# gusanagy/Hybrid-Diffusion-Underwater-Atmopheric-Image-Enhancement

Hardware: AMD Instinct MI355X
Metric: denoising-steps/sec (256x256, T=1000) (higher is better)
Workload: dtype f32 (tensors and accumulation fp32; every operand of the attention contractions as 2xfp16 pieces -- scores: a balance per product term, four terms at d_head 16 / three at d_head 32; P.V: three terms -- and of the 3x3 convs behind GroupNorm likewise (other 3x3 convs: 3xbf16 pieces), on the 16-bit MFM

## Files before the change

### hybrid-diffusion-underwater-atmopheric-image-enhancement_amd/csrc/conv3x3_x3.hip

```cpp
#include <stdlib.h>

#include <type_traits>

#include "common.h"
#include "conv_x3.h"
#include "device.h"

using namespace hdiff;

namespace {

constexpr int THREADS = 256;
constexpr int PH = 10, PW = 34, PPIX = PH * PW;
constexpr int NSLOT = (4 * PPIX + THREADS - 1) / THREADS;
constexpr int HALF_WORDS = PPIX * 4;
constexpr int PIECE_WORDS = 2 * HALF_WORDS;
constexpr int PSTRIDE = PIECE_WORDS + 8;
constexpr int DUMP_WORD = PIECE_WORDS;


__device__ constexpr int TERM_W[6] = {2, 1, 0, 1, 0, 0};
__device__ constexpr int TERM_X[6] = {0, 1, 2, 0, 1, 0};

template <int NT, bool OUTMAP, bool PAIR, int OCC = 1, bool DROP = false>
__global__ __launch_bounds__(THREADS, OCC) void conv3x3_x3_kernel(const ConvX3K p) {
  constexpr int NP = PAIR ? 2 : 3;
  __shared__ __attribute__((aligned(16))) unsigned sXbuf[2][NP * PSTRIDE];
  extern __shared__ __attribute__((aligned(16))) float sG[];

  const int tid = threadIdx.x, lane = tid & 63, wave = tid >> 6;
  const int l31 = lane & 31, h = lane >> 5;
  const int b = blockIdx.z;
  int tile_id = blockIdx.x, cob = blockIdx.y;
  if ((gridDim.x & 7u) == 0u && gridDim.y > 1u) {
    const unsigned lin = blockIdx.x + gridDim.x * blockIdx.y, per = 8u * gridDim.y;
    const unsigned grp = lin / per, r = lin - grp * per;
    tile_id = (int)(grp * 8u + (r & 7u));
    cob = (int)(r >> 3);
  }
  const int co0 = cob * 64;
  const int tile_y = tile_id / p.tiles_x, tile_x = tile_id - tile_y * p.tiles_x;
  const int vy0 = tile_y * 8, vx0 = tile_x * 32;
  const bool has_gn = p.gn_scale != nullptr;
  const size_t HW = (size_t)p.H * p.W;
  const size_t IHW = (size_t)p.IH * p.IW;
  float xs = 1.0f, xinv = 1.0f;
  if constexpr (PAIR) {
    if (p.absmax_in != nullptr) {
      int e = (int)((p.absmax_in[b] >> 23) & 0xffu) - 127;
      e = e < -100 ? -100 : (e > 127 ? 127 : e);
      xs = __builtin_bit_cast(float, (unsigned)(14 - e + 127) << 23);
      xinv = __builtin_bit_cast(float, (unsigned)(e - 14 + 127) << 23);
    } else {
      xs = p.act_scale[0];
      xinv = p.act_scale[1];
    }
  }
  const float one = p.one;

  int s_goff[NSLOT];
  int s_lds[NSLOT];
  int s_quad[NSLOT];
#pragma unroll
  for (int i = 0; i < NSLOT; ++i) {
    const int e = tid + i * THREADS;
    const int jq = e / PPIX, pos = e - jq * PPIX;
    const int py = pos / PW, px = pos - py * PW;
    const int iy = vy0 - 1 + py, ix = vx0 - 1 + px;
    const bool used = jq < 4;
    s_quad[i] = used ? jq : 3;
    s_lds[i] = used ? (jq >> 1) * HALF_WORDS + pos * 4 + (jq & 1) * 2 : DUMP_WORD;
    const int gy = iy * p.in_s + p.in_oy, gx = ix * p.in_s + p.in_ox;
    s_goff[i] = (used && iy >= 0 && gy < p.IH && ix >= 0 && gx < p.IW) ? gy * p.IW + gx : -1;
  }
  if (has_gn) {
    for (int i = tid; i < 2 * p.Cin; i += THREADS)
      sG[i] = (i < p.Cin) ? p.gn_scale[b * p.Cin + i] : p.gn_shift[b * p.Cin + (i - p.Cin)];
  }

  const int wm = wave & 1, wn = wave >> 1;
  f32x16 acc[4];
#pragma unroll
  for (int nt = 0; nt < 4; ++nt)
#pragma unroll
    for (int r = 0; r < 16; ++r) acc[nt][r] = 0.f;

  constexpr bool XAHEAD = PAIR;
  f32x4 xv[NSLOT], xv2[XAHEAD ? NSLOT : 1];
  unsigned kw[DROP ? 4 : 1];
  unsigned ksh = 0;
  auto fetch_keep = [&](int i, int c0, unsigned tie) {
    if constexpr (DROP) {
      const unsigned hw = (unsigned)IHW;
      unsigned e = (unsigned)(b * p.Cin + c0 + 4 * s_quad[i]) * hw + (unsigned)(s_goff[i] >= 0 ? s_goff[i] : 0);
      asm("" : "+v"(e) : "v"(tie));
      ksh = 0;
#pragma unroll
      for (int k = 0; k < 4; ++k) {
        kw[k] = p.keep_bits[e >> 5];
        ksh |= (e & 31u) << (5 * k);
        e += hw;
      }
    }
  };
  auto issue_loads_to = [&](f32x4 (&dst)[XAHEAD ? NSLOT : 1], int c0) {
    const float* xbase = (c0 < p.C0) ? p.x0 + ((size_t)b * p.C0 + c0) * IHW : p.x1 + ((size_t)b * p.C1 + (c0 - p.C0)) * IHW;
#pragma unroll
    for (int i = 0; i < (XAHEAD ? NSLOT : 0); ++i) {
      const bool ok = s_goff[i] >= 0;
      const float* src = xbase + (size_t)(4 * s_quad[i]) * IHW + (ok ? s_goff[i] : 0);
      const float v0 = src[0], v1 = src[IHW], v2 = src[2 * IHW], v3 = src[3 * IHW];
      dst[i] = f32x4{ok ? v0 : 0.f, ok ? v1 : 0.f, ok ? v2 : 0.f, ok ? v3 : 0.f};
    }
  };
  auto issue_loads = [&](int c0) {
    const float* xbase = (c0 < p.C0) ? p.x0 + ((size_t)b * p.C0 + c0) * IHW : p.x1 + ((size_t)b * p.C1 + (c0 - p.C0)) * IHW;
#pragma unroll
    for (int i = 0; i < NSLOT; ++i) {
      const bool ok = s_goff[i] >= 0;
      const float* src = xbase + (size_t)(4 * s_quad[i]) * IHW + (ok ? s_goff[i] : 0);
      const float v0 = src[0], v1 = src[IHW], v2 = src[2 * IHW], v3 = src[3 * IHW];
      xv[i] = f32x4{ok ? v0 : 0.f, ok ? v1 : 0.f, ok ? v2 : 0.f, ok ? v3 : 0.f};
    }
  };
  auto stage_slot = [&](auto gn_tag, int i, int c0, unsigned* sX) {
    constexpr bool GN = decltype(gn_tag)::value;
    f32x4 v = xv[i];
    if (GN) {
      const int ci = c0 + 4 * s_quad[i];
      const f32x4 sc = *reinterpret_cast<const f32x4*>(&sG[ci]);
      const f32x4 sh = *reinterpret_cast<const f32x4*>(&sG[p.Cin + ci]);
      const bool inside = s_goff[i] >= 0;
#pragma unroll
      for (int k = 0; k < 4; ++k) {
        if constexpr (DROP) {
          const bool kept = (kw[k] >> ((ksh >> (5 * k)) & 31u)) & 1u;
          v[k] = (inside && kept) ? swish_fast(fmaf(v[k], sc[k], sh[k])) * p.inv_keep : 0.f;
        } else {
          v[k] = inside ? swish_fast(fmaf(v[k], sc[k], sh[k])) : 0.f;
        }
      }
      if constexpr (DROP) {
        const unsigned tie = __builtin_bit_cast(unsigned, v[0]);
        if (i + 1 < NSLOT) fetch_keep(i + 1, c0, tie);
        else fetch_keep(0, c0 + 16 < p.Cin ? c0 + 16 : c0, tie);
      }
    }
    if constexpr (PAIR) {
      unsigned a0, a1, c0w, c1w;
      split2(v[0] * xs, v[1] * xs, one, a0, a1);
      split2(v[2] * xs, v[3] * xs, one, c0w, c1w);
      if (HDIFF_MUTANT & 1) { a1 &= 0xffe0ffe0u; c1w &= 0xffe0ffe0u; }
      *reinterpret_cast<u32x2*>(&sX[s_lds[i]]) = u32x2{a0, c0w};
      *reinterpret_cast<u32x2*>(&sX[PSTRIDE + s_lds[i]]) = u32x2{a1, c1w};
    } else {
      unsigned a0, a1, a2, c0w, c1w, c2w;
      split3(v[0], v[1], a0, a1, a2);
      split3(v[2], v[3], c0w, c1w, c2w);
      *reinterpret_cast<u32x2*>(&sX[s_lds[i]]) = u32x2{a0, c0w};
      *reinterpret_cast<u32x2*>(&sX[PSTRIDE + s_lds[i]]) = u32x2{a1, c1w};
      *reinterpret_cast<u32x2*>(&sX[2 * PSTRIDE + s_lds[i]]) = u32x2{a2, c2w};
    }
  };
  auto store_staged = [&](auto gn_tag, int c0, unsigned* sX) {
#pragma unroll
    for (int i = 0; i < NSLOT; ++i) stage_slot(gn_tag, i, c0, sX);
  };

  int boff[4];
#pragma unroll
  for (int nt = 0; nt < 4; ++nt) boff[nt] = h * HALF_WORDS + ((wn * 4 + nt) * PW + l31) * 4;
  const unsigned* wlane = p.wp3 + ((size_t)(co0 + wm * 32 + l31) * 8 + h * 4);
  const size_t w_piece = (size_t)p.CoutPad * 8;
  const size_t w_tap = NP * w_piece, w_chunk = NT * w_tap;

  auto load_w = [&](u32x4 (&wa)[NP], int chunk, int tap) {
    const unsigned* wb = wlane + (size_t)chunk * w_chunk + (size_t)tap * w_tap;
#pragma unroll
    for (int pc = 0; pc < NP; ++pc) wa[pc] = *reinterpret_cast<const u32x4*>(wb + pc * w_piece);
  };
  auto load_x = [&](u32x4 (&xp)[NP], const unsigned* sX, int tap, int nt) {
    const int toff = p.tap_off[tap];
#pragma unroll
    for (int pc = 0; pc < NP; ++pc) xp[pc] = *reinterpret_cast<const u32x4*>(&sX[pc * PSTRIDE + boff[nt] + toff]);
  };
  auto mma_unit = [&](const u32x4 (&wa)[NP], const u32x4 (&xp)[NP], int nt) {
    if constexpr (PAIR) {
      acc[nt] = mfma_f16(wa[1], xp[0], acc[nt]);
      acc[nt] = mfma_f16(wa[0], xp[1], acc[nt]);
      acc[nt] = mfma_f16(wa[0], xp[0], acc[nt]);
    } else {
#pragma unroll
      for (int t = 0; t < 6; ++t)
        if (!((HDIFF_MUTANT & 1) && TERM_W[t] == 0 && TERM_X[t] == 2)) acc[nt] = mfma_bf16(wa[TERM_W[t]], xp[TERM_X[t]], acc[nt]);
    }
  };

  constexpr bool WSTREAM = (NT % 3 == 0);
  u32x4 w[3][NP];
  auto chunk = [&](auto gn_tag, auto more_tag, int c, int nchunks) {
    constexpr bool more = decltype(more_tag)::value;
    const unsigned* sX = sXbuf[c & 1];
    unsigned* sNext = sXbuf[(c + 1) & 1];
    u32x4 xp[2][NP];
    if (XAHEAD && c + 2 < nchunks) issue_loads_to(xv2, (c + 2) * 16);
    if (!WSTREAM || c == 0) {
      load_w(w[0], c, 0);
      load_w(w[1], c, 1);
    }
    load_x(xp[0], sX, 0, 0);
#pragma unroll
    for (int tap = 0; tap < NT; ++tap) {
      if (tap + 2 < NT) load_w(w[(tap + 2) % 3], c, tap + 2);
      else if (WSTREAM && more) load_w(w[(tap + 2) % 3], c + 1, tap + 2 - NT);
#pragma unroll
      for (int nt = 0; nt < 4; ++nt) {
        const int u = tap * 4 + nt;
        if (u + 1 < 4 * NT) load_x(xp[(u + 1) & 1], sX, (u + 1) / 4, (u + 1) % 4);
        mma_unit(w[tap % 3], xp[u & 1], nt);
      }
      if (more && tap < NSLOT) stage_slot(gn_tag, tap, (c + 1) * 16, sNext);
    }
    if (more) {
#pragma unroll
      for (int i = NT; i < NSLOT; ++i) stage_slot(gn_tag, i, (c + 1) * 16, sNext);
    }
    if constexpr (XAHEAD) {
      if (c + 2 < nchunks) {
#pragma unroll
        for (int i = 0; i < NSLOT; ++i) xv[i] = xv2[i];
      }
    } else {
      if (c + 2 < nchunks) issue_loads((c + 2) * 16);
    }
    __syncthreads();
  };

  const int nchunks = p.Cin / 16;
  issue_loads(0);
  fetch_keep(0, 0, 0u);
  __syncthreads();
  if (has_gn) store_staged(std::true_type{}, 0, sXbuf[0]);
  else store_staged(std::false_type{}, 0, sXbuf[0]);
  if (nchunks > 1) issue_loads(16);
  __syncthreads();
  if (has_gn) {
    for (int c = 0; c + 1 < nchunks; ++c) chunk(std::true_type{}, std::true_type{}, c, nchunks);
    chunk(std::true_type{}, std::false_type{}, nchunks - 1, nchunks);
  } else {
    for (int c = 0; c + 1 < nchunks; ++c) chunk(std::false_type{}, std::true_type{}, c, nchunks);
    chunk(std::false_type{}, std::false_type{}, nchunks - 1, nchunks);
  }

  if constexpr (PAIR) {
    const float os = xinv * p.w_scale[1];
#pragma unroll
    for (int nt = 0; nt < 4; ++nt)
#pragma unroll
      for (int r = 0; r < 16; ++r) acc[nt][r] *= os;
  }
  const size_t OHW = OUTMAP ? (size_t)p.OH * p.OW : HW;
  const int osy = OUTMAP ? p.out_sy : 1, ooy = OUTMAP ? p.out_oy : 0, osx = OUTMAP ? p.out_sx : 1, oox = OUTMAP ? p.out_ox : 0;
  const int OW = OUTMAP ? p.OW : p.W;
  const bool track = p.absmax_out != nullptr;
  unsigned amax = 0u;
  auto post_absmax = [&]() {
    if (!track) return;
#pragma unroll
    for (int o = 32; o > 0; o >>= 1) {
      const unsigned other = (unsigned)__shfl_xor((int)amax, o, 64);
      amax = other > amax ? other : amax;
    }
    if (lane == 0) atomicMax(&p.absmax_out[b], amax);
  };
  if (co0 + 64 <= p.Cout && vy0 + 8 <= p.H && vx0 + 32 <= p.W) {
    float add[16];
#pragma unroll
    for (int r = 0; r < 16; ++r) {
      const int co = co0 + wm * 32 + (r & 3) + 8 * (r >> 2) + 4 * h;
      float a = 0.f;
      if (p.bias) a += p.bias[co];
      if (p.addvec) a += p.addvec[b * p.Cout + co];
      add[r] = a;
    }
    const size_t lane_base = ((size_t)b * p.Cout + co0 + wm * 32 + 4 * h) * OHW +
                             (size_t)((vy0 + wn * 4) * osy + ooy) * OW + (size_t)(vx0 + l31) * osx + oox;
#pragma unroll
    for (int nt = 0; nt < 4; ++nt) {
      const size_t row = lane_base + (size_t)(nt * osy) * OW;
      float res[16];
      if (p.residual) {
#pragma unroll
        for (int r = 0; r < 16; ++r) res[r] = p.residual[row + (size_t)((r & 3) + 8 * (r >> 2)) * OHW];
      }
      float vv[16];
#pragma unroll
      for (int r = 0; r < 16; ++r) {
        float v;
        if (p.residual_first) v = (acc[nt][r] + res[r]) + add[r];
        else {
          v = acc[nt][r] + add[r];
          if (p.residual) v += res[r];
        }
        p.out[row + (size_t)((r & 3) + 8 * (r >> 2)) * OHW] = v;
        vv[r] = v;
      }
      if (track) {
#pragma unroll
        for (int r = 0; r < 16; ++r) {
          const unsigned vb = __builtin_bit_cast(unsigned, vv[r]) & 0x7fffffffu;
          amax = vb > amax ? vb : amax;
        }
      }
    }
    post_absmax();
    return;
  }
#pragma unroll
  for (int nt = 0; nt < 4; ++nt) {
    const int vy = vy0 + wn * 4 + nt, vx = vx0 + l31;
    if (vy >= p.H || vx >= p.W) continue;
    const size_t pix = (size_t)(vy * osy + ooy) * OW + (size_t)vx * osx + oox;
#pragma unroll
    for (int r = 0; r < 16; ++r) {
      const int co = co0 + wm * 32 + (r & 3) + 8 * (r >> 2) + 4 * h;
      if (co < p.Cout) {
        float a = 0.f;
        if (p.bias) a += p.bias[co];
        if (p.addvec) a += p.addvec[b * p.Cout + co];
        const size_t o = ((size_t)b * p.Cout + co) * OHW + pix;
        float v;
        if (p.residual_first) v = (acc[nt][r] + p.residual[o]) + a;
        else {
          v = acc[nt][r] + a;
          if (p.residual) v += p.residual[o];
        }
        p.out[o] = v;
        if (track) {
          const unsigned vb = __builtin_bit_cast(unsigned, v) & 0x7fffffffu;
          amax = vb > amax ? vb : amax;
        }
      }
    }
  }
  post_absmax();
}

struct PackX3K {
  int mode, Cout, Cin, KH, KW, ntaps, CoutPad;
  int CinPad;
  int ky[9], kx[9];
};
__global__ void pack_conv_weight_x3_kernel(const float* __restrict__ w, unsigned* __restrict__ wp3, const PackX3K q) {
  const size_t n = (size_t)(q.Cin / 16) * q.ntaps * q.CoutPad * 8;
  for (size_t i = (size_t)blockIdx.x * blockDim.x + threadIdx.x; i < n; i += (size_t)gridDim.x * blockDim.x) {
    const int j = (int)(i % 8);
    size_t r = i / 8;
    const int co = (int)(r % q.CoutPad);
    r /= q.CoutPad;
    const int tap = (int)(r % q.ntaps);
    const int chunk = (int)(r / q.ntaps);
    float a = 0.f, c = 0.f;
    if (co < q.Cout) {
      const int ci = chunk * 16 + 2 * j;
      const size_t k = (size_t)q.ky[tap] * q.KW + q.kx[tap], kk = (size_t)q.KH * q.KW;
      if (q.mode == 1) {
        a = w[((size_t)ci * q.Cout + co) * kk + k];
        c = w[((size_t)(ci + 1) * q.Cout + co) * kk + k];
      } else {
        a = w[((size_t)co * q.Cin + ci) * kk + k];
        c = w[((size_t)co * q.Cin + ci + 1) * kk + k];
      }
    }
    unsigned h0, h1, h2;
    split3(a, c, h0, h1, h2);
    const size_t base = ((size_t)(chunk * q.ntaps + tap) * 3) * q.CoutPad * 8 + (size_t)co * 8 + j;
    wp3[base] = h0;
    wp3[base + (size_t)q.CoutPad * 8] = h1;
    wp3[base + 2 * (size_t)q.CoutPad * 8] = h2;
  }
}

__global__ void conv_weight_absmax_kernel(const float* __restrict__ w, size_t n, unsigned* __restrict__ tail) {
  float m = 0.f;
  for (size_t i = (size_t)blockIdx.x * blockDim.x + threadIdx.x; i < n; i += (size_t)gridDim.x * blockDim.x) m = fmaxf(m, fabsf(w[i]));
#pragma unroll
  for (int o = 32; o > 0; o >>= 1) m = fmaxf(m, __shfl_xor(m, o, 64));
  if ((threadIdx.x & 63) == 0) atomicMax(tail, __builtin_bit_cast(unsigned, m));
}
__global__ void pack_conv_weight_h2_kernel(const float* __restrict__ w, unsigned* __restrict__ wp2, unsigned* __restrict__ tail,
                                           const PackX3K q, float one) {
  const size_t n = (size_t)(q.Cin / 16) * q.ntaps * q.CoutPad * 8;
  int e = (int)((tail[0] >> 23) & 0xffu) - 127;
  e = e < -60 ? -60 : (e > 60 ? 60 : e);
  const float sc = __builtin_bit_cast(float, (unsigned)(14 - e + 127) << 23);
  for (size_t i = (size_t)blockIdx.x * blockDim.x + threadIdx.x; i < n; i += (size_t)gridDim.x * blockDim.x) {
    const int j = (int)(i % 8);
    size_t r = i / 8;
    const int co = (int)(r % q.CoutPad);
    r /= q.CoutPad;
    const int tap = (int)(r % q.ntaps);
    const int chunk = (int)(r / q.ntaps);
    float a = 0.f, c = 0.f;
    if (co < q.Cout) {
      const int ci = chunk * 16 + 2 * j;
      const size_t k = (size_t)q.ky[tap] * q.KW + q.kx[tap], kk = (size_t)q.KH * q.KW;
      if (q.mode == 2) {
        a = w[(k * q.CinPad + ci) * q.CoutPad + co];
        c = w[(k * q.CinPad + ci + 1) * q.CoutPad + co];
      } else if (q.mode == 1) {
        a = w[((size_t)ci * q.Cout + co) * kk + k];
        c = w[((size_t)(ci + 1) * q.Cout + co) * kk + k];
      } else {
        a = w[((size_t)co * q.Cin + ci) * kk + k];
        c = w[((size_t)co * q.Cin + ci + 1) * kk + k];
      }
    }
    unsigned h0, h1;
    split2(a * sc, c * sc, one, h0, h1);
    const size_t base = ((size_t)(chunk * q.ntaps + tap) * 2) * q.CoutPad * 8 + (size_t)co * 8 + j;
    wp2[base] = h0;
    wp2[base + (size_t)q.CoutPad * 8] = h1;
  }
  if (blockIdx.x == 0 && threadIdx.x == 0) {
    reinterpret_cast<float*>(tail)[1] = __builtin_bit_cast(float, (unsigned)(e - 14 + 127) << 23);
    reinterpret_cast<float*>(tail)[2] = sc;
    tail[3] = 0u;
  }
}

__global__ void gn_act_scale_kernel(const float* __restrict__ gamma, const float* __restrict__ beta, int C, float sqrt_n1,
                                    float gain, float* __restrict__ out) {
  __shared__ float red[4];
  float m = 0.f;
  for (int i = threadIdx.x; i < C; i += blockDim.x) m = fmaxf(m, fmaf(sqrt_n1, fabsf(gamma[i]), fabsf(beta[i])));
#pragma unroll
  for (int o = 32; o > 0; o >>= 1) m = fmaxf(m, __shfl_xor(m, o, 64));
  if ((threadIdx.x & 63) == 0) red[threadIdx.x >> 6] = m;
  __syncthreads();
  if (threadIdx.x == 0) {
    m = fmaxf(fmaxf(red[0], red[1]), fmaxf(red[2], red[3])) * gain;
    int e = (int)((__builtin_bit_cast(unsigned, m) >> 23) & 0xffu) - 127;
    e = e < -60 ? -60 : (e > 60 ? 60 : e);
    out[0] = __builtin_bit_cast(float, (unsigned)(13 - e + 127) << 23);
    out[1] = __builtin_bit_cast(float, (unsigned)(e - 13 + 127) << 23);
  }
}

}

namespace hdiff {

void launch_conv3x3_x3(const ConvX3K& k, int B, hipStream_t stream) {
  const int tiles_y = cdiv(k.H, 8);
  dim3 grid(k.tiles_x * tiles_y, cdiv(k.Cout, 64), B);
  const size_t dyn = (size_t)2 * k.Cin * sizeof(float);
  const bool outmap = !(k.out_sy == 1 && k.out_oy == 0 && k.out_sx == 1 && k.out_ox == 0 && k.OH == k.H && k.OW == k.W);
  if (k.keep_bits != nullptr) {
    if (k.act_scale != nullptr) hipLaunchKernelGGL((conv3x3_x3_kernel<9, false, true, 2, true>), grid, dim3(THREADS), dyn, stream, k);
    else hipLaunchKernelGGL((conv3x3_x3_kernel<9, false, false, 2, true>), grid, dim3(THREADS), dyn, stream, k);
    return;
  }
  if (k.act_scale != nullptr || k.absmax_in != nullptr) {
    if (k.ntaps == 9 && !outmap) hipLaunchKernelGGL((conv3x3_x3_kernel<9, false, true>), grid, dim3(THREADS), dyn, stream, k);
    else if (k.ntaps == 9) hipLaunchKernelGGL((conv3x3_x3_kernel<9, true, true>), grid, dim3(THREADS), dyn, stream, k);
    else if (k.ntaps == 6 && !outmap) hipLaunchKernelGGL((conv3x3_x3_kernel<6, false, true>), grid, dim3(THREADS), dyn, stream, k);
    else if (k.ntaps == 4 && !outmap) hipLaunchKernelGGL((conv3x3_x3_kernel<4, false, true>), grid, dim3(THREADS), dyn, stream, k);
    else if (k.ntaps == 6) hipLaunchKernelGGL((conv3x3_x3_kernel<6, true, true>), grid, dim3(THREADS), dyn, stream, k);
    else hipLaunchKernelGGL((conv3x3_x3_kernel<4, true, true>), grid, dim3(THREADS), dyn, stream, k);
    return;
  }
  if (k.ntaps == 9 && !outmap) hipLaunchKernelGGL((conv3x3_x3_kernel<9, false, false>), grid, dim3(THREADS), dyn, stream, k);
  else if (k.ntaps == 9) hipLaunchKernelGGL((conv3x3_x3_kernel<9, true, false>), grid, dim3(THREADS), dyn, stream, k);
  else if (k.ntaps == 6) hipLaunchKernelGGL((conv3x3_x3_kernel<6, true, false>), grid, dim3(THREADS), dyn, stream, k);
  else hipLaunchKernelGGL((conv3x3_x3_kernel<4, true, false>), grid, dim3(THREADS), dyn, stream, k);
}

}

static int pack_x3(const float* w, void* wp3, int mode, int Cout, int Cin, int KH, int KW, int ntaps, const int* ky, const int* kx,
                   int CoutPad, hipStream_t stream) {
  PackX3K q{};
  q.mode = mode; q.Cout = Cout; q.Cin = Cin; q.KH = KH; q.KW = KW; q.ntaps = ntaps; q.CoutPad = CoutPad;
  for (int t = 0; t < ntaps; ++t) { q.ky[t] = ky[t]; q.kx[t] = kx[t]; }
  const size_t n = (size_t)(Cin / 16) * ntaps * CoutPad * 8;
  const int blocks = (int)((n + 255) / 256 < 4096 ? (n + 255) / 256 : 4096);
  (void)hipGetLastError();
  hipLaunchKernelGGL(pack_conv_weight_x3_kernel, dim3(blocks), dim3(256), 0, stream, w, (unsigned*)wp3, q);
  HDIFF_CHECK_LAUNCH("pack_conv_weight_x3_kernel");
  return HDIFF_OK;
}

extern "C" int hdiff_pack_conv_weight_x3(const float* w, void* wp3, int Cout, int Cin, int CoutPad, int transposed,
                                         hdiff_stream_t stream) {
  HDIFF_CHECK_ARG(w && wp3, "pack_conv_weight_x3: null pointer");
  HDIFF_CHECK_ARG(Cout > 0 && Cin > 0 && Cin % 16 == 0 && CoutPad >= Cout && CoutPad % 64 == 0,
                  "pack_conv_weight_x3: needs Cin %% 16 == 0 and CoutPad %% 64 == 0 (Cin %d, Cout %d, CoutPad %d)", Cin, Cout, CoutPad);
  int ky[9], kx[9];
  for (int t = 0; t < 9; ++t) {
    ky[t] = transposed ? 2 - t / 3 : t / 3;
    kx[t] = transposed ? 2 - t % 3 : t % 3;
  }
  return pack_x3(w, wp3, transposed ? 1 : 0, Cout, Cin, 3, 3, 9, ky, kx, CoutPad, (hipStream_t)stream);
}

extern "C" int hdiff_pack_conv_weight_h2_words(int Cout, int Cin, int CoutPad, int64_t* words_out) {
  HDIFF_CHECK_ARG(words_out, "pack_conv_weight_h2_words: null pointer");
  HDIFF_CHECK_ARG(Cout > 0 && Cin > 0 && Cin % 16 == 0 && CoutPad >= Cout && CoutPad % 64 == 0,
                  "pack_conv_weight_h2_words: needs Cin %% 16 == 0 and CoutPad %% 64 == 0 (Cin %d, Cout %d, CoutPad %d)", Cin, Cout, CoutPad);
  *words_out = (int64_t)(Cin / 16) * 9 * 2 * CoutPad * 8 + 4;
  return HDIFF_OK;
}

static int pack_h2(const char* who, const float* w, void* wp2, int mode, int Cout, int Cin, int KH, int KW, int ntaps, const int* ky,
                   const int* kx, int CoutPad, hipStream_t stream) {
  PackX3K q{};
  q.mode = mode; q.Cout = Cout; q.Cin = Cin; q.KH = KH; q.KW = KW; q.ntaps = ntaps; q.CoutPad = CoutPad;
  for (int t = 0; t < ntaps; ++t) { q.ky[t] = ky[t]; q.kx[t] = kx[t]; }
  const size_t n = (size_t)(Cin / 16) * ntaps * CoutPad * 8, nw = (size_t)Cout * Cin * KH * KW;
  unsigned* tail = (unsigned*)wp2 + 2 * n;
  const int blocks = (int)((n + 255) / 256 < 4096 ? (n + 255) / 256 : 4096);
  const int mblocks = (int)((nw + 255) / 256 < 1024 ? (nw + 255) / 256 : 1024);
  (void)hipGetLastError();
  if (hipMemsetAsync(tail, 0, 16, stream) != hipSuccess) {
    hdiff::set_error("%s: hipMemsetAsync failed", who);
    return HDIFF_ERR_LAUNCH;
  }
  hipLaunchKernelGGL(conv_weight_absmax_kernel, dim3(mblocks), dim3(256), 0, stream, w, nw, tail);
  HDIFF_CHECK_LAUNCH("conv_weight_absmax_kernel");
  hipLaunchKernelGGL(pack_conv_weight_h2_kernel, dim3(blocks), dim3(256), 0, stream, w, (unsigned*)wp2, tail, q, 1.0f);
  HDIFF_CHECK_LAUNCH("pack_conv_weight_h2_kernel");
  return HDIFF_OK;
}

namespace hdiff {
int s2_plane_taps(int oy, int ox, int* ky, int* kx) {
  int n = 0;
  for (int y = oy; y < 5; y += 2)
    for (int x = ox; x < 5; x += 2) { ky[n] = y; kx[n] = x; ++n; }
  return n;
}
}

extern "C" int hdiff_pack_conv_weight_h2_s2_words(int Cout, int Cin, int CoutPad, int64_t* words_out) {
  HDIFF_CHECK_ARG(words_out, "pack_conv_weight_h2_s2_words: null pointer");
  HDIFF_CHECK_ARG(Cout > 0 && Cin > 0 && Cin % 16 == 0 && CoutPad >= Cout && CoutPad % 64 == 0,
                  "pack_conv_weight_h2_s2_words: needs Cin %% 16 == 0 and CoutPad %% 64 == 0 (Cin %d, Cout %d, CoutPad %d)", Cin, Cout,
                  CoutPad);
  *words_out = (int64_t)(Cin / 16) * 25 * 2 * CoutPad * 8 + 4;
  return HDIFF_OK;
}

extern "C" int hdiff_pack_conv_weight_h2_s2(const float* wp, void* wp2, int Cout, int Cin, int CinPad, int CoutPad, hdiff_stream_t stream) {
  HDIFF_CHECK_ARG(wp && wp2, "pack_conv_weight_h2_s2: null pointer");
  HDIFF_CHECK_ARG(Cout > 0 && Cin > 0 && Cin % 16 == 0 && CinPad >= Cin && CinPad % 8 == 0 && CoutPad >= Cout && CoutPad % 64 == 0,
                  "pack_conv_weight_h2_s2: needs Cin %% 16 == 0, CinPad %% 8 == 0 and CoutPad %% 64 == 0 (Cin %d, CinPad %d, Cout %d, CoutPad %d)",
                  Cin, CinPad, Cout, CoutPad);
  const size_t per_tap = (size_t)(Cin / 16) * 2 * CoutPad * 8, nw = (size_t)25 * CinPad * CoutPad;
  unsigned* tail = (unsigned*)wp2 + 25 * per_tap;
  const int mblocks = (int)((nw + 255) / 256 < 1024 ? (nw + 255) / 256 : 1024);
  (void)hipGetLastError();
  if (hipMemsetAsync(tail, 0, 16, (hipStream_t)stream) != hipSuccess) {
    hdiff::set_error("pack_conv_weight_h2_s2: hipMemsetAsync failed");
    return HDIFF_ERR_LAUNCH;
  }
  hipLaunchKernelGGL(conv_weight_absmax_kernel, dim3(mblocks), dim3(256), 0, (hipStream_t)stream, wp, nw, tail);
  HDIFF_CHECK_LAUNCH("conv_weight_absmax_kernel");
  size_t taps_before = 0;
  for (int g = 0; g < 4; ++g) {
    PackX3K q{};
    q.mode = 2; q.Cout = Cout; q.Cin = Cin; q.KH = 5; q.KW = 5; q.CoutPad = CoutPad; q.CinPad = CinPad;
    q.ntaps = hdiff::s2_plane_taps(g >> 1, g & 1, q.ky, q.kx);
    const size_t n = per_tap / 2 * q.ntaps;
    const int blocks = (int)((n + 255) / 256 < 4096 ? (n + 255) / 256 : 4096);
    hipLaunchKernelGGL(pack_conv_weight_h2_kernel, dim3(blocks), dim3(256), 0, (hipStream_t)stream, wp, (unsigned*)wp2 + taps_before * per_tap,
                       tail, q, 1.0f);
    HDIFF_CHECK_LAUNCH("pack_conv_weight_h2_kernel");
    taps_before += q.ntaps;
  }
  return HDIFF_OK;
}

extern "C" int hdiff_pack_conv_weight_h2(const float* w, void* wp2, int Cout, int Cin, int CoutPad, hdiff_stream_t stream) {
  HDIFF_CHECK_ARG(w && wp2, "pack_conv_weight_h2: null pointer");
  HDIFF_CHECK_ARG(Cout > 0 && Cin > 0 && Cin % 16 == 0 && CoutPad >= Cout && CoutPad % 64 == 0,
                  "pack_conv_weight_h2: needs Cin %% 16 == 0 and CoutPad %% 64 == 0 (Cin %d, Cout %d, CoutPad %d)", Cin, Cout, CoutPad);
  int ky[9], kx[9];
  for (int t = 0; t < 9; ++t) { ky[t] = t / 3; kx[t] = t % 3; }
  return pack_h2("pack_conv_weight_h2", w, wp2, 0, Cout, Cin, 3, 3, 9, ky, kx, CoutPad, (hipStream_t)stream);
}

extern "C" int hdiff_pack_conv_weight_h2_taps_words(int Cout, int Cin, int CoutPad, int ntaps, int64_t* words_out) {
  HDIFF_CHECK_ARG(words_out, "pack_conv_weight_h2_taps_words: null pointer");
  HDIFF_CHECK_ARG(Cout > 0 && Cin > 0 && Cin % 16 == 0 && CoutPad >= Cout && CoutPad % 64 == 0,
                  "pack_conv_weight_h2_taps_words: needs Cin %% 16 == 0 and CoutPad %% 64 == 0 (Cin %d, Cout %d, CoutPad %d)", Cin, Cout,
                  CoutPad);
  HDIFF_CHECK_ARG(ntaps >= 1 && ntaps <= 9, "pack_conv_weight_h2_taps_words: ntaps %d out of range", ntaps);
  *words_out = (int64_t)(Cin / 16) * ntaps * 2 * CoutPad * 8 + 4;
  return HDIFF_OK;
}

extern "C" int hdiff_pack_conv_weight_h2_taps(const float* w, void* wp2, int mode, int Cout, int Cin, int KH, int KW, int ntaps,
                                              const int* tap_ky, const int* tap_kx, int CoutPad, hdiff_stream_t stream) {
  HDIFF_CHECK_ARG(w && wp2 && tap_ky && tap_kx, "pack_conv_weight_h2_taps: null pointer");
  HDIFF_CHECK_ARG(Cout > 0 && Cin > 0 && Cin % 16 == 0 && CoutPad >= Cout && CoutPad % 64 == 0 && (mode == 0 || mode == 1),
                  "pack_conv_weight_h2_taps: needs Cin %% 16 == 0, CoutPad %% 64 == 0, mode 0 / 1 (Cin %d, Cout %d, CoutPad %d, mode %d)",
                  Cin, Cout, CoutPad, mode);
  HDIFF_CHECK_ARG(ntaps >= 1 && ntaps <= 9 && KH > 0 && KW > 0, "pack_conv_weight_h2_taps: ntaps %d out of range", ntaps);
  for (int t = 0; t < ntaps; ++t)
    HDIFF_CHECK_ARG(tap_ky[t] >= 0 && tap_ky[t] < KH && tap_kx[t] >= 0 && tap_kx[t] < KW,
                    "pack_conv_weight_h2_taps: tap %d reads kernel element (%d, %d) of a %d x %d kernel", t, tap_ky[t], tap_kx[t], KH, KW);
  return pack_h2("pack_conv_weight_h2_taps", w, wp2, mode, Cout, Cin, KH, KW, ntaps, tap_ky, tap_kx, CoutPad, (hipStream_t)stream);
}

extern "C" int hdiff_gn_act_scale(const float* gamma, const float* beta, int C, int64_t group_elems, float gain, float* out2,
                                  hdiff_stream_t stream) {
  HDIFF_CHECK_ARG(gamma && beta && out2, "gn_act_scale: null pointer");
  HDIFF_CHECK_ARG(C > 0 && group_elems > 0 && gain >= 1.0f && gain <= 1024.0f, "gn_act_scale: bad sizes (C %d, gain %g)", C, (double)gain);
  (void)hipGetLastError();
  hipLaunchKernelGGL(gn_act_scale_kernel, dim3(1), dim3(256), 0, (hipStream_t)stream, gamma, beta, C,
                     sqrtf((float)(group_elems > 1 ? group_elems - 1 : 1)), gain, out2);
  HDIFF_CHECK_LAUNCH("gn_act_scale_kernel");
  return HDIFF_OK;
}

extern "C" int hdiff_pack_conv_weight_x3_taps(const float* w, void* wp3, int mode, int Cout, int Cin, int KH, int KW, int ntaps,
                                              const int* tap_ky, const int* tap_kx, int CoutPad, hdiff_stream_t stream) {
  HDIFF_CHECK_ARG(w && wp3 && tap_ky && tap_kx, "pack_conv_weight_x3_taps: null pointer");
  HDIFF_CHECK_ARG(Cout > 0 && Cin > 0 && Cin % 16 == 0 && CoutPad >= Cout && CoutPad % 64 == 0 && (mode == 0 || mode == 1),
                  "pack_conv_weight_x3_taps: needs Cin %% 16 == 0, CoutPad %% 64 == 0, mode 0 / 1 (Cin %d, Cout %d, CoutPad %d, mode %d)",
                  Cin, Cout, CoutPad, mode);
  HDIFF_CHECK_ARG(ntaps >= 1 && ntaps <= 9 && KH > 0 && KW > 0, "pack_conv_weight_x3_taps: ntaps %d out of range", ntaps);
  for (int t = 0; t < ntaps; ++t)
    HDIFF_CHECK_ARG(tap_ky[t] >= 0 && tap_ky[t] < KH && tap_kx[t] >= 0 && tap_kx[t] < KW,
                    "pack_conv_weight_x3_taps: tap %d reads kernel element (%d, %d) of a %d x %d kernel", t, tap_ky[t], tap_kx[t], KH, KW);
  return pack_x3(w, wp3, mode, Cout, Cin, KH, KW, ntaps, tap_ky, tap_kx, CoutPad, (hipStream_t)stream);
}
```

Measured before the change: 2.998.

## Add 128-output-channel, 4-row workgroup tile for fp16-pair 3x3 convs

Adds a templated tile shape in which each workgroup covers 128 output channels over 4 rows instead of 64 channels over 8 rows. The four waves are split along output channels only. Whenever Cout is a multiple of 128, the fp16-pair conv path uses this shape. Each staged input tile is then reused by twice as many output channels, which lowers activation loads and LDS staging per output. In exchange, the halo overhead per tile rises (6 of 4 rows instead of 10 of 8), each block reads twice the weights, and the grid shape changes.

```diff
diff --git a/hybrid-diffusion-underwater-atmopheric-image-enhancement_amd/csrc/conv3x3_x3.hip b/hybrid-diffusion-underwater-atmopheric-image-enhancement_amd/csrc/conv3x3_x3.hip
--- a/hybrid-diffusion-underwater-atmopheric-image-enhancement_amd/csrc/conv3x3_x3.hip
+++ b/hybrid-diffusion-underwater-atmopheric-image-enhancement_amd/csrc/conv3x3_x3.hip
@@ -11,19 +11,28 @@
 namespace {
 
 constexpr int THREADS = 256;
-constexpr int PH = 10, PW = 34, PPIX = PH * PW;
-constexpr int NSLOT = (4 * PPIX + THREADS - 1) / THREADS;
-constexpr int HALF_WORDS = PPIX * 4;
-constexpr int PIECE_WORDS = 2 * HALF_WORDS;
-constexpr int PSTRIDE = PIECE_WORDS + 8;
-constexpr int DUMP_WORD = PIECE_WORDS;
+constexpr int PW = 34;
+template <int COB>
+struct Tile {
+  static_assert(COB == 64 || COB == 128, "workgroup tile: 64 or 128 output channels");
+  static constexpr int ROWS = COB == 64 ? 8 : 4;
+  static constexpr int PH = ROWS + 2, PPIX = PH * PW;
+  static constexpr int NSLOT = (4 * PPIX + THREADS - 1) / THREADS;
+  static constexpr int HALF_WORDS = PPIX * 4;
+  static constexpr int PIECE_WORDS = 2 * HALF_WORDS;
+  static constexpr int PSTRIDE = PIECE_WORDS + 8;
+  static constexpr int DUMP_WORD = PIECE_WORDS;
+};
 
 
 __device__ constexpr int TERM_W[6] = {2, 1, 0, 1, 0, 0};
 __device__ constexpr int TERM_X[6] = {0, 1, 2, 0, 1, 0};
 
-template <int NT, bool OUTMAP, bool PAIR, int OCC = 1, bool DROP = false>
+template <int NT, bool OUTMAP, bool PAIR, int OCC = 1, bool DROP = false, int COB = 64>
 __global__ __launch_bounds__(THREADS, OCC) void conv3x3_x3_kernel(const ConvX3K p) {
+  static_assert(COB == 64 || (PAIR && !DROP), "the 128-channel tile: fp16 pairs without dropout only");
+  using T = Tile<COB>;
+  constexpr int ROWS = T::ROWS, PPIX = T::PPIX, NSLOT = T::NSLOT, HALF_WORDS = T::HALF_WORDS, PSTRIDE = T::PSTRIDE, DUMP_WORD = T::DUMP_WORD;
   constexpr int NP = PAIR ? 2 : 3;
   __shared__ __attribute__((aligned(16))) unsigned sXbuf[2][NP * PSTRIDE];
   extern __shared__ __attribute__((aligned(16))) float sG[];
@@ -38,9 +47,9 @@
     tile_id = (int)(grp * 8u + (r & 7u));
     cob = (int)(r >> 3);
   }
-  const int co0 = cob * 64;
+  const int co0 = cob * COB;
   const int tile_y = tile_id / p.tiles_x, tile_x = tile_id - tile_y * p.tiles_x;
-  const int vy0 = tile_y * 8, vx0 = tile_x * 32;
+  const int vy0 = tile_y * ROWS, vx0 = tile_x * 32;
   const bool has_gn = p.gn_scale != nullptr;
   const size_t HW = (size_t)p.H * p.W;
   const size_t IHW = (size_t)p.IH * p.IW;
@@ -78,7 +87,7 @@
       sG[i] = (i < p.Cin) ? p.gn_scale[b * p.Cin + i] : p.gn_shift[b * p.Cin + (i - p.Cin)];
   }
 
-  const int wm = wave & 1, wn = wave >> 1;
+  const int wm = COB == 64 ? (wave & 1) : wave, wn = COB == 64 ? (wave >> 1) : 0;
   f32x16 acc[4];
 #pragma unroll
   for (int nt = 0; nt < 4; ++nt)
@@ -273,7 +282,7 @@
     }
     if (lane == 0) atomicMax(&p.absmax_out[b], amax);
   };
-  if (co0 + 64 <= p.Cout && vy0 + 8 <= p.H && vx0 + 32 <= p.W) {
+  if (co0 + COB <= p.Cout && vy0 + ROWS <= p.H && vx0 + 32 <= p.W) {
     float add[16];
 #pragma unroll
     for (int r = 0; r < 16; ++r) {
@@ -462,6 +471,16 @@
     return;
   }
   if (k.act_scale != nullptr || k.absmax_in != nullptr) {
+    if (k.Cout % 128 == 0) {
+      const dim3 grid128(k.tiles_x * cdiv(k.H, 4), k.Cout / 128, B);
+      if (k.ntaps == 9 && !outmap) hipLaunchKernelGGL((conv3x3_x3_kernel<9, false, true, 1, false, 128>), grid128, dim3(THREADS), dyn, stream, k);
+      else if (k.ntaps == 9) hipLaunchKernelGGL((conv3x3_x3_kernel<9, true, true, 1, false, 128>), grid128, dim3(THREADS), dyn, stream, k);
+      else if (k.ntaps == 6 && !outmap) hipLaunchKernelGGL((conv3x3_x3_kernel<6, false, true, 1, false, 128>), grid128, dim3(THREADS), dyn, stream, k);
+      else if (k.ntaps == 4 && !outmap) hipLaunchKernelGGL((conv3x3_x3_kernel<4, false, true, 1, false, 128>), grid128, dim3(THREADS), dyn, stream, k);
+      else if (k.ntaps == 6) hipLaunchKernelGGL((conv3x3_x3_kernel<6, true, true, 1, false, 128>), grid128, dim3(THREADS), dyn, stream, k);
+      else hipLaunchKernelGGL((conv3x3_x3_kernel<4, true, true, 1, false, 128>), grid128, dim3(THREADS), dyn, stream, k);
+      return;
+    }
     if (k.ntaps == 9 && !outmap) hipLaunchKernelGGL((conv3x3_x3_kernel<9, false, true>), grid, dim3(THREADS), dyn, stream, k);
     else if (k.ntaps == 9) hipLaunchKernelGGL((conv3x3_x3_kernel<9, true, true>), grid, dim3(THREADS), dyn, stream, k);
     else if (k.ntaps == 6 && !outmap) hipLaunchKernelGGL((conv3x3_x3_kernel<6, false, true>), grid, dim3(THREADS), dyn, stream, k);
```

New measurement: 3.020 (median of 6 runs). About the same (+0.7%).
